# isl-org/Open3D-ML

Hardware: AMD Instinct MI355X
Metric: point-cloud frames/sec (RandLA-Net SemanticKITTI inference: H2D + kNN pyramid + forward) (higher is better)
Workload: dtype f32

## Files before the change

open3d-ml_amd/csrc/grid.h:

```cpp
#pragma once
#include <hip/hip_runtime.h>
#include <stdint.h>

namespace ml3d {

constexpr int GRID_CAP = 8;
constexpr int GRID_SLACK = 64;
constexpr int GRID_LEVELS = 5;

struct Segs {
    const int64_t* splits;
    int64_t stride;
    int64_t n_uniform;
    int batch;
};

struct GridSeg {
    float lo[3];
    float c, inv_c;
    float margin;
    int dims[3];
    int cell_base;
    int n;
    int sorted_base;
    float c0;
    int dims0[3];
    float ext[3];
    float dim_est;
    int probe_stride;
};

struct GridView {
    const GridSeg* segs;
    const int* cell_start;
    const float4* sorted;
    int batch;
};

struct GridWs {
    GridSeg* segs;
    unsigned* bbox;
    unsigned* occ;
    unsigned* bitmap;
    int* cells;
    int* block_sums;
    float4* sorted;
    int64_t total_cells;
    int64_t bitmap_words;
    int64_t n_total;
    int batch;
};

constexpr int GRID_SORTED_SLACK = 4;
size_t grid_ws_bytes(int64_t n_total, int64_t batch);
bool grid_ws_carve(void* ws, size_t bytes, int64_t n_total, int64_t batch, GridWs* out);
int grid_build(const float* points, Segs segs, const GridWs& ws, float target_occ, hipStream_t stream);
int grid_build_derived(const float* points, Segs segs, const GridWs& ws, const GridWs& parent, hipStream_t stream);
int grid_build_fixed(const float* points, Segs segs, const GridWs& ws, float cell, hipStream_t stream);
int bbox_compute(const float* points, Segs segs, int64_t n_total, unsigned* bbox, unsigned* occ_scratch,
                 hipStream_t stream);
int scan_inclusive_i32(int* a, int64_t n, int* block_sums, hipStream_t stream);

void zero_async(void* ptr, size_t bytes, hipStream_t stream);

__device__ __forceinline__ unsigned f2ord(float f) {
    unsigned u = __float_as_uint(f);
    return (u & 0x80000000u) ? ~u : (u | 0x80000000u);
}
__device__ __forceinline__ float ord2f(unsigned u) {
    return __uint_as_float((u & 0x80000000u) ? (u & 0x7fffffffu) : ~u);
}

__device__ __forceinline__ void wave_sync() {
    __threadfence_block();
    __builtin_amdgcn_wave_barrier();
}

__device__ __forceinline__ void wave_lds_sync() {
    __builtin_amdgcn_fence(__ATOMIC_RELEASE, "wavefront");
    __builtin_amdgcn_wave_barrier();
    __builtin_amdgcn_fence(__ATOMIC_ACQUIRE, "wavefront");
}


__device__ __forceinline__ float fmax_raw(float a, float b) { return __builtin_amdgcn_fmed3f(a, b, 3.0e38f); }

__device__ __forceinline__ int wave_inclusive_scan(int v) {
    const int lane = threadIdx.x & 63;
#pragma unroll
    for (int o = 1; o < 64; o <<= 1) {
        int u = __shfl_up(v, o);
        if (lane >= o) v += u;
    }
    return v;
}
__device__ __forceinline__ int wave_sum(int v) {
#pragma unroll
    for (int o = 32; o > 0; o >>= 1) v += __shfl_xor(v, o);
    return v;
}

__device__ __forceinline__ void block_sync_lds() {
    __builtin_amdgcn_fence(__ATOMIC_RELEASE, "workgroup", "local");
    __builtin_amdgcn_s_barrier();
    __builtin_amdgcn_fence(__ATOMIC_ACQUIRE, "workgroup", "local");
}

inline GridView grid_view(const GridWs& ws) {
    GridView v;
    v.segs = ws.segs;
    v.cell_start = ws.cells;
    v.sorted = ws.sorted;
    v.batch = ws.batch;
    return v;
}


__device__ __forceinline__ int64_t seg_begin_global(const Segs& S, int s) {
    return S.splits ? S.splits[s] : (int64_t)s * S.stride;
}
__device__ __forceinline__ int64_t seg_begin_packed(const Segs& S, int s) {
    return S.splits ? S.splits[s] : (int64_t)s * S.n_uniform;
}
__device__ __forceinline__ int64_t seg_len(const Segs& S, int s) {
    return S.splits ? (S.splits[s + 1] - S.splits[s]) : S.n_uniform;
}
__device__ __forceinline__ void seg_locate(const Segs& S, int64_t packed, int& s, int64_t& local) {
    if (!S.splits) {
        s = (int)(packed / S.n_uniform);
        local = packed - (int64_t)s * S.n_uniform;
        return;
    }
    int lo = 0, hi = S.batch;
    while (hi - lo > 1) {
        int mid = (lo + hi) >> 1;
        if (S.splits[mid] <= packed) lo = mid; else hi = mid;
    }
    s = lo;
    local = packed - S.splits[lo];
}
// ... 42 lines not shown
```

open3d-ml_amd/csrc/grid.hip:

```cpp
#include "grid.h"

#include <math.h>

namespace ml3d {

static inline size_t align_up(size_t x) { return (x + 255) & ~(size_t)255; }

static void grid_sizes(int64_t n_total, int64_t batch, int64_t* total_cells, int64_t* bitmap_words,
                       int64_t* n_blocks) {
    *total_cells = (int64_t)GRID_CAP * n_total + (int64_t)GRID_SLACK * batch;
    *bitmap_words = (*total_cells + 31) / 32 + batch;
    *n_blocks = (*total_cells + 2 + 1023) / 1024 + 1;
}

size_t grid_ws_bytes(int64_t n_total, int64_t batch) {
    int64_t tc, bw, nb;
    grid_sizes(n_total, batch, &tc, &bw, &nb);
    size_t b = 0;
    b += align_up(sizeof(GridSeg) * (size_t)batch);
    b += align_up(sizeof(unsigned) * 6 * (size_t)batch);
    b += align_up(sizeof(unsigned) * GRID_LEVELS * (size_t)batch);
    b += align_up(sizeof(unsigned) * GRID_LEVELS * (size_t)bw);
    b += align_up(sizeof(int) * (size_t)(tc + 2));
    b += align_up(sizeof(int) * (size_t)nb);
// ... 221 lines not shown
        const int64_t last = first + blockDim.x - 1 < total ? first + blockDim.x - 1 : total - 1;
        s0 = (int)(first / per); s1 = (int)(last / per);
    } else {
        const int64_t last = first + blockDim.x - 1 < n_total ? first + blockDim.x - 1 : n_total - 1;
        seg_locate_wave(S, first, s0, l0);
        seg_locate_wave(S, last, s1, l1);
    }
    const bool one_item = (s0 == s1);
    if (threadIdx.x < GRID_LEVELS) cnt[threadIdx.x] = 0u;
    __syncthreads();
    const int64_t i = first + threadIdx.x;
    bool valid;
    int s = s0; int64_t local = l0 + threadIdx.x;
    if (dense_stride > 0) {
        s = (int)(i / per);
        local = (i - (int64_t)s * per) * dense_stride;
        valid = s < S.batch && local < S.n_uniform;
        if (!valid) s = s0;
    } else {
        valid = i < n_total;
        if (valid && !one_item) seg_locate(S, i, s, local);
    }
    int cx = 0, cy = 0, cz = 0;
    const GridSeg* g = &segs[s];
    valid = valid && (local % g->probe_stride == 0);
    if (valid) {
        const float* p = pts + 3 * (seg_begin_global(S, s) + local);
        float inv = 1.0f / g->c0;
        cx = cell_coord(p[0], g->lo[0], inv, g->dims0[0]);
        cy = cell_coord(p[1], g->lo[1], inv, g->dims0[1]);
        cz = cell_coord(p[2], g->lo[2], inv, g->dims0[2]);
    }
    const int64_t bit_base = (int64_t)g->cell_base + 32 * (int64_t)s;
    for (int l = 0; l < GRID_LEVELS; ++l) {
        bool fresh = false;
        if (valid) {
            int dx = ((g->dims0[0] - 1) >> l) + 1, dy = ((g->dims0[1] - 1) >> l) + 1;
            int64_t id = (cx >> l) + (int64_t)dx * ((cy >> l) + (int64_t)dy * (cz >> l));
            int64_t bit = bit_base + id;
            unsigned m = 1u << (unsigned)(bit & 31);
            unsigned old = atomicOr(&bitmap[(int64_t)l * bitmap_words + (bit >> 5)], m);
            fresh = !(old & m);
        }
        if (one_item) {
            unsigned long long b = __ballot(fresh);
            if ((threadIdx.x & 63) == 0 && b) atomicAdd(&cnt[l], (unsigned)__popcll(b));
        } else if (fresh) {
            atomicAdd(&occ[GRID_LEVELS * s + l], 1u);
        }
    }
    __syncthreads();
    if (one_item && threadIdx.x < GRID_LEVELS && cnt[threadIdx.x])
        atomicAdd(&occ[GRID_LEVELS * s0 + threadIdx.x], cnt[threadIdx.x]);
}

__device__ __forceinline__ float occ_of_lam(float lam) { return lam / (1.0f - expf(-lam)); }
__device__ __forceinline__ float lam_of_occ(float m) {
    if (m <= 1.0005f) return 1.0e-3f;
    float lo = 1.0e-3f, hi = 64.0f;
    if (m >= hi) return m;
    for (int it = 0; it < 40; ++it) {
        float mid = 0.5f * (lo + hi);
        if (occ_of_lam(mid) < m) lo = mid; else hi = mid;
    }
    return 0.5f * (lo + hi);
}

__device__ __forceinline__ void finish_grid(GridSeg& g, float c, int64_t cap) {
    float emax = fmaxf(g.ext[0], fmaxf(g.ext[1], g.ext[2]));
    int d[3] = {1, 1, 1};
    if (emax > 0.f) {
        for (int it = 0; it < 200; ++it) {
            if (dims_fit(g.ext, c, cap, d)) break;
            c *= 1.1f;
        }
    } else {
        c = 1.0f;
    }
    g.c = c;
    g.inv_c = 1.0f / c;
    for (int a = 0; a < 3; ++a) g.dims[a] = d[a];
}

__global__ void grid_setup1(const unsigned* occ, GridSeg* segs, int batch, float target) {
    int s = blockIdx.x * blockDim.x + threadIdx.x;
    if (s >= batch) return;
    GridSeg g = segs[s];
    int64_t n = g.n;
    float emax = fmaxf(g.ext[0], fmaxf(g.ext[1], g.ext[2]));
    int64_t cap = (int64_t)GRID_CAP * n + GRID_SLACK;
    float c = g.c0;
    if (n > 0 && emax > 0.f) {
        const float n_probe = (float)((n + g.probe_stride - 1) / g.probe_stride);
        const float lam_goal = lam_of_occ(target) / (float)g.probe_stride;
        float lam_prev = 0.f, lam_cur = 0.f;
        int lsel = -1;
        for (int l = 0; l < GRID_LEVELS; ++l) {
            unsigned cnt = occ[GRID_LEVELS * s + l];
            lam_cur = lam_of_occ(n_probe / (float)(cnt > 0u ? cnt : 1u));
            if (lam_cur >= lam_goal) { lsel = l; break; }
            lam_prev = lam_cur;
        }
        if (lsel == 0) {
            c = g.c0;
        } else if (lsel > 0) {
            float D = fminf(fmaxf(log2f(lam_cur / lam_prev), 1.0f), 3.0f);
            g.dim_est = D;
            c = g.c0 * (float)(1 << (lsel - 1)) * powf(lam_goal / lam_prev, 1.0f / D);
        } else {
            c = g.c0 * (float)(1 << (GRID_LEVELS - 1));
            if (n <= 64) c = emax * 2.0f;
        }
    }
    finish_grid(g, c, cap);
    segs[s] = g;
}

__global__ void grid_setup_derived(Segs S, const GridSeg* parent, GridSeg* segs, int batch) {
    int s = blockIdx.x * blockDim.x + threadIdx.x;
    if (s >= batch) return;
    GridSeg g = parent[s];
    int64_t n = seg_len(S, s);
    int64_t pb = seg_begin_packed(S, s);
    float ratio = n > 0 ? (float)g.n / (float)n : 1.0f;
    float c = g.c * powf(fmaxf(ratio, 1.0f), 1.0f / g.dim_est);
    g.n = (int)n;
    g.sorted_base = (int)pb;
    g.cell_base = (int)(GRID_CAP * pb + (int64_t)GRID_SLACK * s);
    if (n <= 64) c = fmaxf(g.ext[0], fmaxf(g.ext[1], g.ext[2])) * 2.0f;
    finish_grid(g, c, (int64_t)GRID_CAP * n + GRID_SLACK);
    segs[s] = g;
}

__device__ __forceinline__ int point_cell(const GridSeg* g, float x, float y, float z) {
    int cx = cell_coord(x, g->lo[0], g->inv_c, g->dims[0]);
    int cy = cell_coord(y, g->lo[1], g->inv_c, g->dims[1]);
    int cz = cell_coord(z, g->lo[2], g->inv_c, g->dims[2]);
    return g->cell_base + cx + g->dims[0] * (cy + g->dims[1] * cz);
}

__global__ void grid_hist(const float* __restrict__ pts, Segs S, int64_t n_total,
                          const GridSeg* __restrict__ segs, int* cells) {
    int64_t i = (int64_t)blockIdx.x * blockDim.x + threadIdx.x;
    if (i >= n_total) return;
    int s; int64_t local;
    seg_locate(S, i, s, local);
    const float* p = pts + 3 * (seg_begin_global(S, s) + local);
    int cid = point_cell(&segs[s], p[0], p[1], p[2]);
    atomicAdd(&cells[cid + 2], 1);
}

constexpr int SCAN_TILE = 4096;


__global__ void __launch_bounds__(256) scan_block_sums(const int* __restrict__ a, int64_t n, int* block_sums) {
    __shared__ int ws[4];
    const int64_t base = (int64_t)blockIdx.x * SCAN_TILE;
    int v = 0;
#pragma unroll
    for (int j = 0; j < SCAN_TILE / 256; ++j) {
        int64_t i = base + j * 256 + threadIdx.x;
        if (i < n) v += a[i];
    }
    v = wave_sum(v);
    if ((threadIdx.x & 63) == 0) ws[threadIdx.x >> 6] = v;
    __syncthreads();
    if (threadIdx.x == 0) block_sums[blockIdx.x] = ws[0] + ws[1] + ws[2] + ws[3];
}

__global__ void __launch_bounds__(1024) scan_sums(int* block_sums, int64_t nb) {
    __shared__ int wsum[16];
    const int t = threadIdx.x;
    const int64_t per = (nb + 1023) / 1024;
    const int64_t lo = (int64_t)t * per, hi = lo + per < nb ? lo + per : nb;
    int s = 0;
    for (int64_t i = lo; i < hi; ++i) s += block_sums[i];
    int incl = wave_inclusive_scan(s);
    if ((t & 63) == 63) wsum[t >> 6] = incl;
    __syncthreads();
    int carry = 0;
    for (int w = 0; w < (t >> 6); ++w) carry += wsum[w];
    int run = carry + incl - s;
    for (int64_t i = lo; i < hi; ++i) {
        int v = block_sums[i];
        block_sums[i] = run;
        run += v;
    }
}

__global__ void __launch_bounds__(256) scan_final(int* a, int64_t n, const int* __restrict__ block_sums) {
    __shared__ int ws[4];
    const int lane = threadIdx.x & 63, wv = threadIdx.x >> 6;
    const int64_t base = (int64_t)blockIdx.x * SCAN_TILE + (int64_t)wv * 1024;
    int v[16], tot = 0;
#pragma unroll
    for (int r = 0; r < 16; ++r) {
        int64_t i = base + r * 64 + lane;
        v[r] = i < n ? a[i] : 0;
        tot += v[r];
    }
    tot = wave_sum(tot);
    if (lane == 0) ws[wv] = tot;
    __syncthreads();
    int carry = block_sums[blockIdx.x];
    for (int w = 0; w < wv; ++w) carry += ws[w];
#pragma unroll
    for (int r = 0; r < 16; ++r) {
        int incl = wave_inclusive_scan(v[r]) + carry;
        int64_t i = base + r * 64 + lane;
        if (i < n) a[i] = incl;
        carry = __shfl(incl, 63);
    }
}

// ... 74 lines not shown
    return 0;
}

static int grid_sort(const float* points, Segs S, const GridWs& ws, hipStream_t stream) {
    int64_t n = ws.n_total;
    int nb = (int)((n + 255) / 256);
    if (n > 0) {
        hipLaunchKernelGGL(grid_hist, dim3(nb), dim3(256), 0, stream, points, S, n, ws.segs, ws.cells);
        ML3D_LAUNCH_CHECK();
        if (scan_inclusive_i32(ws.cells + 2, ws.total_cells, ws.block_sums, stream)) return -3;
        hipLaunchKernelGGL(grid_scatter, dim3(nb), dim3(256), 0, stream, points, S, n, ws.segs, ws.cells,
                           ws.sorted);
        ML3D_LAUNCH_CHECK();
    }
    return 0;
}


int grid_build(const float* points, Segs S, const GridWs& ws, float target_occ, hipStream_t stream) {
    int64_t n = ws.n_total;
    int B = ws.batch;
    if (B <= 0) return 0;
    if (target_occ <= 0.f) target_occ = 4.0f;
    int sb = (B + 63) / 64;
    zero_async(ws.bitmap, (size_t)((char*)(ws.cells + ws.total_cells + 2) - (char*)ws.bitmap), stream);
    hipLaunchKernelGGL(grid_bbox_init, dim3(sb), dim3(64), 0, stream, ws.bbox, ws.occ, B);
    ML3D_LAUNCH_CHECK();
    if (n > 0) {
        int nb4 = (int)((n + 1023) / 1024);
        hipLaunchKernelGGL(grid_bbox, dim3(nb4), dim3(256), 0, stream, points, S, n, ws.bbox);
        ML3D_LAUNCH_CHECK();
    }
    hipLaunchKernelGGL(grid_setup0, dim3(sb), dim3(64), 0, stream, S, ws.bbox, ws.segs, B);
    ML3D_LAUNCH_CHECK();
    int nb = (int)((n + 255) / 256);
    if (n > 0) {
        const int dense = (!S.splits && S.n_uniform >= 32768) ? 16 : 0;
        const int nbo = dense ? (int)((((S.n_uniform + dense - 1) / dense) * (int64_t)S.batch + 255) / 256) : nb;
        hipLaunchKernelGGL(grid_occupancy, dim3(nbo), dim3(256), 0, stream, points, S, n, ws.segs, ws.bitmap,
                           ws.bitmap_words, ws.occ, dense);
        ML3D_LAUNCH_CHECK();
    }
    hipLaunchKernelGGL(grid_setup1, dim3(sb), dim3(64), 0, stream, ws.occ, ws.segs, B, target_occ);
    ML3D_LAUNCH_CHECK();
    return grid_sort(points, S, ws, stream);
}

__global__ void grid_setup_fixed(GridSeg* segs, int batch, float cell) {
    int s = blockIdx.x * blockDim.x + threadIdx.x;
    if (s >= batch) return;
    GridSeg g = segs[s];
    float c = cell;
    if (!(c > 0.f)) c = g.c0;
    if (c < g.c0 * 0.5f) c = g.c0 * 0.5f;
    finish_grid(g, c, (int64_t)GRID_CAP * g.n + GRID_SLACK);
    segs[s] = g;
}

int bbox_compute(const float* points, Segs S, int64_t n, unsigned* bbox, unsigned* occ_scratch, hipStream_t stream) {
    int B = S.batch;
    if (B <= 0) return 0;
    hipLaunchKernelGGL(grid_bbox_init, dim3((B + 63) / 64), dim3(64), 0, stream, bbox, occ_scratch, B);
    ML3D_LAUNCH_CHECK();
    if (n > 0) {
        hipLaunchKernelGGL(grid_bbox, dim3((unsigned)((n + 1023) / 1024)), dim3(256), 0, stream, points, S, n, bbox);
        ML3D_LAUNCH_CHECK();
    }
    return 0;
}

int grid_build_fixed(const float* points, Segs S, const GridWs& ws, float cell, hipStream_t stream) {
    int B = ws.batch;
    if (B <= 0) return 0;
    int sb = (B + 63) / 64;
    zero_async(ws.cells, sizeof(int) * (size_t)(ws.total_cells + 2), stream);
    if (bbox_compute(points, S, ws.n_total, ws.bbox, ws.occ, stream)) return -3;
    hipLaunchKernelGGL(grid_setup0, dim3(sb), dim3(64), 0, stream, S, ws.bbox, ws.segs, B);
    ML3D_LAUNCH_CHECK();
    hipLaunchKernelGGL(grid_setup_fixed, dim3(sb), dim3(64), 0, stream, ws.segs, B, cell);
    ML3D_LAUNCH_CHECK();
    return grid_sort(points, S, ws, stream);
}

int grid_build_derived(const float* points, Segs S, const GridWs& ws, const GridWs& parent, hipStream_t stream) {
    int B = ws.batch;
    if (B <= 0) return 0;
    zero_async(ws.cells, sizeof(int) * (size_t)(ws.total_cells + 2), stream);
    hipLaunchKernelGGL(grid_setup_derived, dim3((B + 63) / 64), dim3(64), 0, stream, S, parent.segs, ws.segs, B);
    ML3D_LAUNCH_CHECK();
    return grid_sort(points, S, ws, stream);
}

}
```

open3d-ml_amd/csrc/knn.hip:

```cpp
#include <hip/hip_runtime.h>
#include <stdint.h>
#include <stdlib.h>

#include <gfx950_ops.h>

#include "grid.h"
#include "ml3d_hip.h"

namespace ml3d {

typedef unsigned long long u64;
constexpr u64 KEY_EMPTY = 0x7ff0000000000000ull;

struct QuerySrc {
    const float4* sorted_q;
    const GridSeg* qsegs;
    const float* raw;
    Segs segs;
    int64_t n_total;
};

template <int K>
__device__ __forceinline__ void topk_insert(double (&best)[K], double key) {
    if (key < best[K - 1]) {
// ... 142 lines not shown
        };
        float dk = 3.0e38f;
        int r_in = 0, r = 1;
        if constexpr (MODE == 2) {
#pragma unroll
            for (int j = 0; j < K; ++j) best[j] = H->keys[(size_t)j * H->cap + hslot];
            best1 = H->keys[(size_t)K * H->cap + hslot];
            u64 kth0;
            dk = known_within(kth0);
            r_in = 1; r = 2;
        }
        for (;;) {
            scan_shell<K, SUB>(G, g, qx, qy, qz, cx, cy, cz, r_in, r, dk, best, n_sub, best1);
            bool all;
            const float gd = shell_guard(g, qx, qy, qz, cx, cy, cz, r, all);
            if (all) break;
            u64 kth;
            dk = known_within(kth);
            if (kth != KEY_EMPTY && gd > 0.f && dk < gd * gd * 0.999999f) break;
            if constexpr (MODE == 1) {
                if (r == 1) {
                    const unsigned slot = wave_append(H->count);
                    if (slot < H->cap) {
#pragma unroll
                        for (int j = 0; j < K; ++j) H->keys[(size_t)j * H->cap + slot] = best[j];
                        H->keys[(size_t)K * H->cap + slot] = best1;
                        H->who[slot] = (job << 28) | (uint32_t)t;
                        return;
                    }
                }
            }
            r_in = r;
            if (r < UNIT_SHELLS) { ++r; continue; }
            int rn = r + max(1, r >> 1);
            if (dk < 3.0e38f) {
                const float rad = sqrtf(dk) * 1.00001f + g.margin;
                const int need = max(max(cx - cell_coord(qx - rad, g.lo[0], g.inv_c, g.dims[0]), cell_coord(qx + rad, g.lo[0], g.inv_c, g.dims[0]) - cx),
                                     max(max(cy - cell_coord(qy - rad, g.lo[1], g.inv_c, g.dims[1]), cell_coord(qy + rad, g.lo[1], g.inv_c, g.dims[1]) - cy),
                                         max(cz - cell_coord(qz - rad, g.lo[2], g.inv_c, g.dims[2]), cell_coord(qz + rad, g.lo[2], g.inv_c, g.dims[2]) - cz)));
                rn = max(r + 1, need);
            }
            r = rn;
        }
    }
    int64_t base = index_local ? 0 : seg_begin_global(support_segs, s);
    if (SUB) {
        const u64 k1 = (u64)__double_as_longlong(best1);
        out_sub[out_row] = k1 != KEY_EMPTY ? (int32_t)(unsigned)(k1 & 0xffffffffull) : -1;
    }
    if (K == 16 && k == 16 && !out_d2 && vec_store) {
        struct alignas(16) I4 { int32_t v[4]; };
        I4* dst = reinterpret_cast<I4*>(out_idx + out_row * 16);
#pragma unroll
        for (int qd = 0; qd < 4; ++qd) {
            I4 o;
#pragma unroll
            for (int e = 0; e < 4; ++e) {
                const u64 key = (u64)__double_as_longlong(best[4 * qd + e]);
                o.v[e] = key != KEY_EMPTY ? (int32_t)((int64_t)(unsigned)(key & 0xffffffffull) + base) : -1;
            }
            dst[qd] = o;
        }
        return;
    }
#pragma unroll
    for (int j = 0; j < K; ++j) {
        if (j < k) {
            u64 key = (u64)__double_as_longlong(best[j]);
            bool ok = key != KEY_EMPTY;
            out_idx[out_row * k + j] = ok ? (int32_t)((int64_t)(unsigned)(key & 0xffffffffull) + base) : -1;
            if (out_d2) out_d2[out_row * k + j] = ok ? __uint_as_float((unsigned)(key >> 32)) : __uint_as_float(0x7f800000u);
        }
    }
}

template <int K>
__global__ void __launch_bounds__(256)
knn_query(GridView G, QuerySrc Q, int k, int index_local, Segs support_segs, int32_t* __restrict__ out_idx,
          float* __restrict__ out_d2) {
    knn_one<K, false>(G, Q, k, index_local, support_segs, out_idx, out_d2, (int64_t)blockIdx.x * blockDim.x + threadIdx.x);
}

constexpr int KNN_MAX_JOBS = 8;
struct KnnJob {
    GridView G;
    QuerySrc Q;
    Segs support;
    int32_t* out_idx;
    int32_t* out_sub;
    int n_sub;
    unsigned block_begin;
};
struct KnnJobs {
    KnnJob j[KNN_MAX_JOBS];
    int n;
};

#ifndef KNN_WAVES
#define KNN_WAVES 5
#endif
template <int K, bool SUB, bool HAND>
__global__ void __launch_bounds__(256)
#if KNN_WAVES > 0
ML3D_WAVES_PER_SIMD(KNN_WAVES)
#endif
knn_query_multi(KnnJobs J, int k, int index_local, int vec_store, Handoff H) {
    int ji = 0;
#pragma unroll
    for (int i = 1; i < KNN_MAX_JOBS; ++i)
        if (i < J.n && blockIdx.x >= J.j[i].block_begin) ji = i;
    const KnnJob& jb = J.j[ji];
    knn_one<K, SUB, HAND ? 1 : 0>(jb.G, jb.Q, k, index_local, jb.support, jb.out_idx, nullptr,
                                  (int64_t)(blockIdx.x - jb.block_begin) * blockDim.x + threadIdx.x, jb.n_sub, jb.out_sub, vec_store != 0,
                                  &H, (unsigned)ji);
}

#ifndef KNN_WAVES_HAND
#define KNN_WAVES_HAND 4
#endif
template <int K, bool SUB>
__global__ void __launch_bounds__(256)
ML3D_WAVES_PER_SIMD(KNN_WAVES_HAND)
knn_first(KnnJobs J, int k, int index_local, int vec_store, Handoff H) {
    int ji = 0;
#pragma unroll
    for (int i = 1; i < KNN_MAX_JOBS; ++i)
        if (i < J.n && blockIdx.x >= J.j[i].block_begin) ji = i;
    const KnnJob& jb = J.j[ji];
    knn_one<K, SUB, 1>(jb.G, jb.Q, k, index_local, jb.support, jb.out_idx, nullptr,
                       (int64_t)(blockIdx.x - jb.block_begin) * blockDim.x + threadIdx.x, jb.n_sub, jb.out_sub, vec_store != 0, &H, (unsigned)ji);
}

template <int K, bool SUB>
__global__ void __launch_bounds__(256)
ML3D_WAVES_PER_SIMD(KNN_WAVES_HAND)
knn_continue(KnnJobs J, int k, int index_local, int vec_store, Handoff H) {
    const unsigned have = *H.count;
    const unsigned n = have < H.cap ? have : H.cap;
    const unsigned i = blockIdx.x * blockDim.x + threadIdx.x;
    if (i >= n) return;
    const uint32_t who = H.who[i];
    const KnnJob& jb = J.j[who >> 28];
    knn_one<K, SUB, 2>(jb.G, jb.Q, k, index_local, jb.support, jb.out_idx, nullptr, (int64_t)(who & 0x0fffffffu), jb.n_sub, jb.out_sub,
                       vec_store != 0, &H, who >> 28, i);
}

static int knn_block() { return 64; }

static size_t handoff_bytes(int64_t total_queries) {
    const size_t cap = (size_t)(total_queries * 5 / 8 + 64);
    return 256 + ((cap * 4 + 255) & ~(size_t)255) + 17 * cap * 8 + 256;
}
static Handoff handoff_carve(char* p, int64_t total_queries) {
    Handoff H;
    const size_t cap = (size_t)(total_queries * 5 / 8 + 64);
    p = (char*)(((uintptr_t)p + 255) & ~(uintptr_t)255);
    H.count = (unsigned*)p;  p += 256;
    H.who = (uint32_t*)p;    p += (cap * 4 + 255) & ~(size_t)255;
    H.keys = (double*)p;
    H.cap = (unsigned)cap;
    return H;
}

#ifndef ML3D_KNN_HANDOFF
#define ML3D_KNN_HANDOFF 0
#endif

template <bool SUB>
static int launch_query_multi(KnnJobs& J, int k, int index_local, hipStream_t stream, const Handoff* hand = nullptr) {
    const int T = knn_block();
    unsigned blocks = 0;
    int vec = 1;
    for (int i = 0; i < J.n; ++i) {
        J.j[i].block_begin = blocks;
        blocks += (unsigned)((J.j[i].Q.n_total + T - 1) / T);
        if ((uintptr_t)J.j[i].out_idx & 15) vec = 0;
    }
    if (blocks == 0) return 0;
    Handoff H = {};
    if ((ML3D_KNN_HANDOFF) && hand && k > 8 && k <= 16) {
        H = *hand;
        zero_async(H.count, 16, stream);
        hipLaunchKernelGGL((knn_first<16, SUB>), dim3(blocks), dim3(T), 0, stream, J, k, index_local, vec, H);
        if (hipGetLastError() != hipSuccess) return ML3D_E_LAUNCH;
        hipLaunchKernelGGL((knn_continue<16, SUB>), dim3((H.cap + T - 1) / T), dim3(T), 0, stream, J, k, index_local, vec, H);
        return hipGetLastError() == hipSuccess ? 0 : ML3D_E_LAUNCH;
    }
    if (k == 1) hipLaunchKernelGGL((knn_query_multi<1, SUB, false>), dim3(blocks), dim3(T), 0, stream, J, k, index_local, vec, H);
    else if (k <= 8) hipLaunchKernelGGL((knn_query_multi<8, SUB, false>), dim3(blocks), dim3(T), 0, stream, J, k, index_local, vec, H);
    else if (k <= 16) hipLaunchKernelGGL((knn_query_multi<16, SUB, false>), dim3(blocks), dim3(T), 0, stream, J, k, index_local, vec, H);
    else if (k <= 32) hipLaunchKernelGGL((knn_query_multi<32, SUB, false>), dim3(blocks), dim3(T), 0, stream, J, k, index_local, vec, H);
    else if (k <= 64) hipLaunchKernelGGL((knn_query_multi<64, SUB, false>), dim3(blocks), dim3(T), 0, stream, J, k, index_local, vec, H);
    else return ML3D_E_UNSUPPORTED;
    return hipGetLastError() == hipSuccess ? 0 : ML3D_E_LAUNCH;
}

static int launch_query(const GridView& G, const QuerySrc& Q, int k, int index_local, Segs support_segs,
                        int32_t* out_idx, float* out_d2, hipStream_t stream) {
    if (Q.n_total <= 0) return 0;
    dim3 grid((unsigned)((Q.n_total + 255) / 256)), block(256);
    if (k == 1)
        hipLaunchKernelGGL(knn_query<1>, grid, block, 0, stream, G, Q, k, index_local, support_segs, out_idx, out_d2);
    else if (k <= 8)
        hipLaunchKernelGGL(knn_query<8>, grid, block, 0, stream, G, Q, k, index_local, support_segs, out_idx, out_d2);
    else if (k <= 16)
        hipLaunchKernelGGL(knn_query<16>, grid, block, 0, stream, G, Q, k, index_local, support_segs, out_idx, out_d2);
    else if (k <= 32)
        hipLaunchKernelGGL(knn_query<32>, grid, block, 0, stream, G, Q, k, index_local, support_segs, out_idx, out_d2);
    else if (k <= 64)
        hipLaunchKernelGGL(knn_query<64>, grid, block, 0, stream, G, Q, k, index_local, support_segs, out_idx, out_d2);
    else
        return ML3D_E_UNSUPPORTED;
    return hipGetLastError() == hipSuccess ? 0 : ML3D_E_LAUNCH;
}

__global__ void order_from_grid(const float4* __restrict__ sorted, int64_t n_total, int64_t n_per_item,
                                int32_t* __restrict__ out) {
    const int64_t i = (int64_t)blockIdx.x * blockDim.x + threadIdx.x;
    if (i >= n_total) return;
    out[i] = (int32_t)((i / n_per_item) * n_per_item + (int64_t)__float_as_int(sorted[i].w));
}

static constexpr float tuning_occ() { return 0.f; }

}

using namespace ml3d;

extern "C" int ml3d_abi_version(void) { return ML3D_ABI_VERSION; }

extern "C" size_t ml3d_knn_workspace_bytes(int64_t n_points, int64_t n_queries, int64_t batch) {
    (void)n_queries;
    return grid_ws_bytes(n_points, batch);
}

extern "C" int ml3d_knn_search(const float* points, const int64_t* points_row_splits, const float* queries,
                               const int64_t* queries_row_splits, int64_t batch, int64_t n_points,
                               int64_t n_queries, int k, int index_local, int32_t* out_index,
                               float* out_dist2, void* workspace, size_t workspace_bytes, void* stream) {
    if (!points_row_splits || !queries_row_splits || batch <= 0 || k <= 0 || n_points < 0 || n_queries < 0 ||
        n_points > 0x7fffffffll / GRID_CAP - 4096 || n_queries > 0x7fffffffll)
        return ML3D_E_INVALID;
    if (k > 64) return ML3D_E_UNSUPPORTED;
    if (n_queries == 0) return 0;
    if (!out_index || (n_points > 0 && !points) || !queries) return ML3D_E_INVALID;
    GridWs ws;
    if (!grid_ws_carve(workspace, workspace_bytes, n_points, batch, &ws)) return ML3D_E_WORKSPACE;
    hipStream_t st = (hipStream_t)stream;
    Segs ps = {points_row_splits, 0, 0, (int)batch};
    Segs qs = {queries_row_splits, 0, 0, (int)batch};
    int rc = grid_build(points, ps, ws, tuning_occ(), st);
    if (rc) return ML3D_E_LAUNCH;
    GridView G = grid_view(ws);
    QuerySrc Q;
    bool self = (queries == points) && (queries_row_splits == points_row_splits) && (n_queries == n_points);
    Q.sorted_q = self ? ws.sorted : nullptr;
    Q.qsegs = ws.segs;
    Q.raw = queries;
    Q.segs = qs;
    Q.n_total = n_queries;
    return launch_query(G, Q, k, index_local, ps, out_index, out_dist2, st);
}

static int pyramid_sizes(int64_t n0, int num_layers, const int32_t* ratios, int64_t* n ) {
    n[0] = n0;
    for (int l = 0; l < num_layers; ++l) {
        if (ratios[l] <= 0) return -1;
        n[l + 1] = n[l] / ratios[l];
    }
    return 0;
}

extern "C" size_t ml3d_randla_pyramid_workspace_bytes(int64_t batch, int64_t n0, int num_layers,
                                                      const int32_t* ratios_host) {
    if (num_layers <= 0 || num_layers > KNN_MAX_JOBS || !ratios_host) return 0;
    int64_t n[17];
    if (pyramid_sizes(n0, num_layers, ratios_host, n)) return 0;
    size_t b = 0;
    int64_t total = 0;
    for (int l = 0; l < num_layers; ++l) { b += grid_ws_bytes(n[l] * batch, batch) + 256; total += n[l] * batch; }
    return b + handoff_bytes(total);
}

extern "C" int ml3d_randla_knn_pyramid(const float* points, int64_t batch, int64_t n0, int num_layers,
                                       const int32_t* ratios_host, int k, int32_t* const* neighbor_idx_host,
                                       int32_t* const* interp_idx_host, void* workspace, size_t workspace_bytes,
                                       void* stream) {
    return ml3d_randla_knn_pyramid_traced(points, batch, n0, num_layers, ratios_host, k, neighbor_idx_host,
                                          interp_idx_host, workspace, workspace_bytes, stream, nullptr);
}

extern "C" int ml3d_randla_knn_pyramid_traced(const float* points, int64_t batch, int64_t n0, int num_layers,
                                              const int32_t* ratios_host, int k,
                                              int32_t* const* neighbor_idx_host, int32_t* const* interp_idx_host,
                                              void* workspace, size_t workspace_bytes, void* stream,
                                              const ml3d_trace* tr) {
    return ml3d_randla_knn_pyramid_ordered(points, batch, n0, num_layers, ratios_host, k, neighbor_idx_host,
                                           interp_idx_host, nullptr, workspace, workspace_bytes, stream, tr);
}

extern "C" int ml3d_randla_knn_pyramid_ordered(const float* points, int64_t batch, int64_t n0, int num_layers,
                                               const int32_t* ratios_host, int k,
                                               int32_t* const* neighbor_idx_host, int32_t* const* interp_idx_host,
                                               int32_t* const* tile_order_host, void* workspace,
                                               size_t workspace_bytes, void* stream, const ml3d_trace* tr) {
    auto tb = [&](int tag) { for (const ml3d_trace* r = tr; r; r = r->next) if (r->tag == tag && r->ev_start) (void)hipEventRecord((hipEvent_t)r->ev_start, (hipStream_t)stream); };
    auto te = [&](int tag) { for (const ml3d_trace* r = tr; r; r = r->next) if (r->tag == tag && r->ev_stop) (void)hipEventRecord((hipEvent_t)r->ev_stop, (hipStream_t)stream); };
    if (!points || batch <= 0 || n0 <= 0 || num_layers <= 0 || num_layers > KNN_MAX_JOBS || !ratios_host || k <= 0 ||
        !neighbor_idx_host || !interp_idx_host)
        return ML3D_E_INVALID;
    if (k > 64) return ML3D_E_UNSUPPORTED;
    int64_t n[17];
    if (pyramid_sizes(n0, num_layers, ratios_host, n)) return ML3D_E_INVALID;
    if (n0 * batch > 0x7fffffffll / GRID_CAP - 4096) return ML3D_E_INVALID;
    if (workspace_bytes < ml3d_randla_pyramid_workspace_bytes(batch, n0, num_layers, ratios_host))
        return ML3D_E_WORKSPACE;
    hipStream_t st = (hipStream_t)stream;
    GridWs ws[17];
    char* p = (char*)workspace;
    for (int l = 0; l < num_layers; ++l) {
        size_t bytes = grid_ws_bytes(n[l] * batch, batch) + 256;
        if (!grid_ws_carve(p, bytes, n[l] * batch, batch, &ws[l])) return ML3D_E_WORKSPACE;
        p += bytes;
    }
    float occ = tuning_occ();
    for (int l = 0; l < num_layers; ++l) {
        if (n[l] == 0) continue;
        Segs S = {nullptr, n0, n[l], (int)batch};
        tb(100 + l);
        if (l == 0 ? grid_build(points, S, ws[l], occ, st) : grid_build_derived(points, S, ws[l], ws[0], st))
            return ML3D_E_LAUNCH;
        if (tile_order_host && tile_order_host[l]) {
            const int64_t nt = n[l] * batch;
            hipLaunchKernelGGL(order_from_grid, dim3((unsigned)((nt + 255) / 256)), dim3(256), 0, st, ws[l].sorted, nt, n[l],
                               tile_order_host[l]);
            if (hipGetLastError() != hipSuccess) return ML3D_E_LAUNCH;
        }
        te(100 + l);
    }
    KnnJobs Jk;
    Jk.n = 0;
    for (int l = 0; l < num_layers; ++l) {
        if (n[l] == 0) continue;
        Segs S = {nullptr, n0, n[l], (int)batch};
        QuerySrc Q;
        Q.sorted_q = ws[l].sorted;
        Q.qsegs = ws[l].segs;
        Q.raw = points;
        Q.segs = S;
        Q.n_total = n[l] * batch;
        KnnJob& a = Jk.j[Jk.n++];
        a.G = grid_view(ws[l]); a.Q = Q; a.support = S; a.out_idx = neighbor_idx_host[l]; a.block_begin = 0;
        a.out_sub = interp_idx_host[l];
        a.n_sub = (int)n[l + 1];
    }
    int64_t total_q = 0;
    for (int l = 0; l < num_layers; ++l) total_q += n[l] * batch;
    const Handoff hand = handoff_carve(p, total_q);
    tb(0);
    int rc = launch_query_multi<true>(Jk, k, 1, st, &hand);
    te(0);
    return rc;
}

#include <hip/hip_fp16.h>

#include "sort.h"

namespace ml3d {

__global__ void center_keys(const float* __restrict__ pts, int64_t n, double cx, double cy, double cz,
                            const float* __restrict__ cdev, u64* __restrict__ keys, uint32_t* __restrict__ vals) {
    const int64_t i = (int64_t)blockIdx.x * blockDim.x + threadIdx.x;
    if (i >= n) return;
    if (cdev) { cx = (double)cdev[0]; cy = (double)cdev[1]; cz = (double)cdev[2]; }
    const double dx = (double)pts[3 * i] - cx, dy = (double)pts[3 * i + 1] - cy, dz = (double)pts[3 * i + 2] - cz;
    const double d2 = (dx * dx + dy * dy) + dz * dz;
    keys[i] = (u64)__double_as_longlong(d2);
    vals[i] = (uint32_t)i;
}

__global__ void center_take(const u64* __restrict__ keys, const uint32_t* __restrict__ vals, int64_t k,
                            int32_t* __restrict__ out_idx, double* __restrict__ out_d2) {
    const int64_t i = (int64_t)blockIdx.x * blockDim.x + threadIdx.x;
    if (i >= k) return;
    out_idx[i] = (int32_t)vals[i];
    if (out_d2) out_d2[i] = __longlong_as_double((long long)keys[i]);
}

__global__ void __launch_bounds__(256)
vote_update(const float* __restrict__ logits, const int32_t* __restrict__ inds, int64_t n, int C, float smooth,
            __half* __restrict__ probs, int64_t n_cloud) {
    const int lane = threadIdx.x & 63;
    const int64_t i = (int64_t)blockIdx.x * 4 + (threadIdx.x >> 6);
    if (i >= n) return;
    const float* row = logits + i * C;
    float mx = -3.0e38f;
    for (int c = lane; c < C; c += 64) mx = fmaxf(mx, row[c]);
#pragma unroll
    for (int o = 32; o > 0; o >>= 1) mx = fmaxf(mx, __shfl_xor(mx, o));
    float sum = 0.f;
    for (int c = lane; c < C; c += 64) sum += expf(row[c] - mx);
#pragma unroll
    for (int o = 32; o > 0; o >>= 1) sum += __shfl_xor(sum, o);
    const int64_t dst = inds[i];
    if (dst < 0 || dst >= n_cloud) return;
    const __half hs = __float2half(smooth);
    const float w_new = 1.0f - smooth;
    for (int c = lane; c < C; c += 64) {
        const float p = expf(row[c] - mx) / sum;
        const __half old = probs[dst * C + c];
        const __half keep = __float2half(__half2float(hs) * __half2float(old));
        probs[dst * C + c] = __float2half(__half2float(keep) + w_new * p);
    }
}

__global__ void __launch_bounds__(256)
argmax_rows(const float* __restrict__ scores, int64_t n, int C, uint8_t* __restrict__ out) {
    const int64_t i = (int64_t)blockIdx.x * blockDim.x + threadIdx.x;
    if (i >= n) return;
    const float* row = scores + i * C;
    float best = row[0];
    int arg = 0;
    for (int c = 1; c < C; ++c) {
        const float v = row[c];
        if ((v > best || v != v) && !(best != best)) { best = v; arg = c; }
    }
    out[i] = (uint8_t)arg;
}

__global__ void __launch_bounds__(64)
argmax_rows_lds(const float* __restrict__ scores, int64_t n, int C, uint8_t* __restrict__ out) {
    __shared__ __attribute__((aligned(16))) float tile[64 * 32];
    const int64_t r0 = (int64_t)blockIdx.x * 64;
    const int rows = (int)((n - r0) < 64 ? (n - r0) : 64);
    const int64_t f0 = r0 * C;
    const int total = rows * C;
    const float* src = scores + f0;
    const int mis = (int)(f0 & 3);
    const int head = mis ? 4 - mis : 0;
    for (int e = threadIdx.x; e < head && e < total; e += 64) tile[e] = src[e];
    const int n4 = total > head ? (total - head) / 4 : 0;
    const float4* s4 = reinterpret_cast<const float4*>(src + head);
// ... 226 lines not shown
```

Measured before the change: 7558.

## Build all kNN pyramid grids in one fused multi-level pass

Measured after the change: 7562 (median of 2 runs). Within noise of the previous version (+0.0%).

```diff
diff --git a/open3d-ml_amd/csrc/grid.h b/open3d-ml_amd/csrc/grid.h
--- a/open3d-ml_amd/csrc/grid.h
+++ b/open3d-ml_amd/csrc/grid.h
@@ -55,7 +55,9 @@
 size_t grid_ws_bytes(int64_t n_total, int64_t batch);
 bool grid_ws_carve(void* ws, size_t bytes, int64_t n_total, int64_t batch, GridWs* out);
 int grid_build(const float* points, Segs segs, const GridWs& ws, float target_occ, hipStream_t stream);
-int grid_build_derived(const float* points, Segs segs, const GridWs& ws, const GridWs& parent, hipStream_t stream);
+constexpr int GRID_MAX_LEVELS = 8;
+int grid_build_pyramid(const float* points, const int64_t* n, int num_levels, int batch, const GridWs* ws,
+                       int32_t* const* tile_order, float target_occ, hipStream_t stream);
 int grid_build_fixed(const float* points, Segs segs, const GridWs& ws, float cell, hipStream_t stream);
 int bbox_compute(const float* points, Segs segs, int64_t n_total, unsigned* bbox, unsigned* occ_scratch,
                  hipStream_t stream);
diff --git a/open3d-ml_amd/csrc/grid.hip b/open3d-ml_amd/csrc/grid.hip
--- a/open3d-ml_amd/csrc/grid.hip
+++ b/open3d-ml_amd/csrc/grid.hip
@@ -327,10 +327,7 @@
     for (int a = 0; a < 3; ++a) g.dims[a] = d[a];
 }
 
-__global__ void grid_setup1(const unsigned* occ, GridSeg* segs, int batch, float target) {
-    int s = blockIdx.x * blockDim.x + threadIdx.x;
-    if (s >= batch) return;
-    GridSeg g = segs[s];
+__device__ __forceinline__ void setup1_item(const unsigned* occ, GridSeg& g, int s, float target) {
     int64_t n = g.n;
     float emax = fmaxf(g.ext[0], fmaxf(g.ext[1], g.ext[2]));
     int64_t cap = (int64_t)GRID_CAP * n + GRID_SLACK;
@@ -358,15 +355,17 @@
         }
     }
     finish_grid(g, c, cap);
-    segs[s] = g;
-}
-
-__global__ void grid_setup_derived(Segs S, const GridSeg* parent, GridSeg* segs, int batch) {
+}
+
+__global__ void grid_setup1(const unsigned* occ, GridSeg* segs, int batch, float target) {
     int s = blockIdx.x * blockDim.x + threadIdx.x;
     if (s >= batch) return;
-    GridSeg g = parent[s];
-    int64_t n = seg_len(S, s);
-    int64_t pb = seg_begin_packed(S, s);
+    GridSeg g = segs[s];
+    setup1_item(occ, g, s, target);
+    segs[s] = g;
+}
+
+__device__ __forceinline__ void derived_item(GridSeg& g, int64_t n, int64_t pb, int s) {
     float ratio = n > 0 ? (float)g.n / (float)n : 1.0f;
     float c = g.c * powf(fmaxf(ratio, 1.0f), 1.0f / g.dim_est);
     g.n = (int)n;
@@ -374,7 +373,6 @@
     g.cell_base = (int)(GRID_CAP * pb + (int64_t)GRID_SLACK * s);
     if (n <= 64) c = fmaxf(g.ext[0], fmaxf(g.ext[1], g.ext[2])) * 2.0f;
     finish_grid(g, c, (int64_t)GRID_CAP * n + GRID_SLACK);
-    segs[s] = g;
 }
 
 __device__ __forceinline__ int point_cell(const GridSeg* g, float x, float y, float z) {
@@ -615,13 +613,214 @@
     return grid_sort(points, S, ws, stream);
 }
 
-int grid_build_derived(const float* points, Segs S, const GridWs& ws, const GridWs& parent, hipStream_t stream) {
-    int B = ws.batch;
-    if (B <= 0) return 0;
-    zero_async(ws.cells, sizeof(int) * (size_t)(ws.total_cells + 2), stream);
-    hipLaunchKernelGGL(grid_setup_derived, dim3((B + 63) / 64), dim3(64), 0, stream, S, parent.segs, ws.segs, B);
-    ML3D_LAUNCH_CHECK();
-    return grid_sort(points, S, ws, stream);
-}
-
-}
+struct GridLevels {
+    GridSeg* segs[GRID_MAX_LEVELS];
+    int* cells[GRID_MAX_LEVELS];
+    float4* sorted[GRID_MAX_LEVELS];
+    int32_t* order[GRID_MAX_LEVELS];
+    int n[GRID_MAX_LEVELS];
+    unsigned zero_begin[GRID_MAX_LEVELS];
+    unsigned zero_per[GRID_MAX_LEVELS];
+    int nl, batch;
+};
+
+__device__ __forceinline__ int seg_used_cells(const GridSeg& g) { return g.dims[0] * g.dims[1] * g.dims[2]; }
+
+__global__ void grid_setup_levels(GridLevels L, const unsigned* occ, float target) {
+    int s = blockIdx.x * blockDim.x + threadIdx.x;
+    if (s >= L.batch) return;
+    GridSeg g0 = L.segs[0][s];
+    setup1_item(occ, g0, s, target);
+    L.segs[0][s] = g0;
+    for (int l = 1; l < L.nl; ++l) {
+        GridSeg g = g0;
+        derived_item(g, L.n[l], (int64_t)s * L.n[l], s);
+        L.segs[l][s] = g;
+    }
+}
+
+constexpr int ZERO_WORDS = 4096;
+__global__ void __launch_bounds__(256)
+grid_zero_bitmap(const GridSeg* __restrict__ segs, unsigned* __restrict__ bitmap, int64_t bitmap_words, unsigned chunks) {
+    const unsigned sl = blockIdx.x / chunks, chunk = blockIdx.x % chunks;
+    const int s = (int)(sl / GRID_LEVELS), l = (int)(sl % GRID_LEVELS);
+    const GridSeg* g = &segs[s];
+    const int64_t bits = (int64_t)(((g->dims0[0] - 1) >> l) + 1) * (((g->dims0[1] - 1) >> l) + 1) * (((g->dims0[2] - 1) >> l) + 1);
+    const int64_t bit_base = (int64_t)g->cell_base + 32 * (int64_t)s;
+    const int64_t w0 = bit_base >> 5, w1 = (bit_base + bits - 1) >> 5;
+    const int64_t first = w0 + (int64_t)chunk * ZERO_WORDS;
+    if (first > w1) return;
+    unsigned* p = bitmap + (int64_t)l * bitmap_words;
+#pragma unroll
+    for (int j = 0; j < ZERO_WORDS / 256; ++j) {
+        const int64_t w = first + j * 256 + threadIdx.x;
+        if (w <= w1) p[w] = 0u;
+    }
+}
+
+__global__ void __launch_bounds__(256) grid_zero_cells(GridLevels L) {
+    int l = 0;
+#pragma unroll
+    for (int i = 1; i < GRID_MAX_LEVELS; ++i)
+        if (i < L.nl && blockIdx.x >= L.zero_begin[i]) l = i;
+    const unsigned rel = blockIdx.x - L.zero_begin[l];
+    const int s = (int)(rel / L.zero_per[l]);
+    const int chunk = (int)(rel % L.zero_per[l]);
+    const GridSeg* g = &L.segs[l][s];
+    const int len = seg_used_cells(*g) + 2;
+    if (chunk * ZERO_WORDS >= len) return;
+    int* a = L.cells[l] + g->cell_base;
+#pragma unroll
+    for (int j = 0; j < ZERO_WORDS / 1024; ++j) {
+        const int w = chunk * ZERO_WORDS + 4 * (j * 256 + (int)threadIdx.x);
+        if (w + 4 <= len) {
+            *(uint4*)(a + w) = make_uint4(0u, 0u, 0u, 0u);
+        } else {
+            for (int q = w; q < len; ++q) a[q] = 0;
+        }
+    }
+}
+
+__global__ void __launch_bounds__(256) grid_hist_levels(const float* __restrict__ pts, GridLevels L) {
+    const int64_t i = (int64_t)blockIdx.x * blockDim.x + threadIdx.x;
+    const int n0 = L.n[0];
+    if (i >= (int64_t)n0 * L.batch) return;
+    const int s = (int)(i / n0), local = (int)(i - (int64_t)s * n0);
+    const float* p = pts + 3 * i;
+    const float x = p[0], y = p[1], z = p[2];
+#pragma unroll
+    for (int l = 0; l < GRID_MAX_LEVELS; ++l)
+        if (l < L.nl && local < L.n[l]) atomicAdd(&L.cells[l][point_cell(&L.segs[l][s], x, y, z) + 2], 1);
+}
+
+__global__ void __launch_bounds__(1024) grid_scan_items(GridLevels L) {
+    __shared__ int ws[16];
+    const int l = blockIdx.x / L.batch, s = blockIdx.x % L.batch;
+    const int lane = threadIdx.x & 63, wv = threadIdx.x >> 6;
+    const GridSeg* g = &L.segs[l][s];
+    const int used = seg_used_cells(*g);
+    const int first_slot = g->sorted_base;
+    int* a = L.cells[l] + g->cell_base + 2;
+    if (threadIdx.x == 0) {
+        int reach = 0;
+        if (s > 0) {
+            const GridSeg* gp = &L.segs[l][s - 1];
+            reach = seg_used_cells(*gp) + 2 - (g->cell_base - gp->cell_base);
+        }
+        if (reach < 1) a[-2] = first_slot;
+        if (reach < 2) a[-1] = first_slot;
+    }
+    const int rows = (used + 1023) / 1024;
+    const int base = wv * rows * 64;
+    int tot = 0;
+    for (int r = 0; r < rows; r += 4) {
+        int v[4];
+#pragma unroll
+        for (int q = 0; q < 4; ++q) {
+            const int i = base + (r + q) * 64 + lane;
+            v[q] = (r + q < rows && i < used) ? a[i] : 0;
+        }
+        tot += (v[0] + v[1]) + (v[2] + v[3]);
+    }
+    tot = wave_sum(tot);
+    if (lane == 0) ws[wv] = tot;
+    __syncthreads();
+    int carry = first_slot;
+    for (int w = 0; w < wv; ++w) carry += ws[w];
+    for (int r = 0; r < rows; r += 4) {
+        int v[4];
+#pragma unroll
+        for (int q = 0; q < 4; ++q) {
+            const int i = base + (r + q) * 64 + lane;
+            v[q] = (r + q < rows && i < used) ? a[i] : 0;
+        }
+#pragma unroll
+        for (int q = 0; q < 4; ++q) {
+            const int i = base + (r + q) * 64 + lane;
+            const int incl = wave_inclusive_scan(v[q]) + carry;
+            if (r + q < rows && i < used) a[i] = incl;
+            carry = __shfl(incl, 63);
+        }
+    }
+}
+
+__global__ void __launch_bounds__(256) grid_scatter_levels(const float* __restrict__ pts, GridLevels L) {
+    const int64_t i = (int64_t)blockIdx.x * blockDim.x + threadIdx.x;
+    const int n0 = L.n[0];
+    if (i >= (int64_t)n0 * L.batch) return;
+    const int s = (int)(i / n0), local = (int)(i - (int64_t)s * n0);
+    const float* p = pts + 3 * i;
+    const float x = p[0], y = p[1], z = p[2];
+    const float4 e = make_float4(x, y, z, __int_as_float(local));
+    int pos[GRID_MAX_LEVELS];
+#pragma unroll
+    for (int l = 0; l < GRID_MAX_LEVELS; ++l)
+        if (l < L.nl && local < L.n[l]) pos[l] = atomicAdd(&L.cells[l][point_cell(&L.segs[l][s], x, y, z) + 1], 1);
+#pragma unroll
+    for (int l = 0; l < GRID_MAX_LEVELS; ++l) {
+        if (l < L.nl && local < L.n[l]) {
+            L.sorted[l][pos[l]] = e;
+            if (L.order[l]) L.order[l][pos[l]] = s * L.n[l] + local;
+        }
+    }
+}
+
+int grid_build_pyramid(const float* points, const int64_t* n, int num_levels, int batch, const GridWs* ws,
+                       int32_t* const* tile_order, float target_occ, hipStream_t stream) {
+    if (batch <= 0 || num_levels <= 0) return 0;
+    if (num_levels > GRID_MAX_LEVELS || n[0] <= 0) return -3;
+    if (target_occ <= 0.f) target_occ = 4.0f;
+    const int B = batch, sb = (B + 63) / 64;
+    const int64_t nt = n[0] * B;
+    GridLevels L;
+    L.nl = num_levels;
+    L.batch = B;
+    unsigned zero_blocks = 0;
+    for (int l = 0; l < GRID_MAX_LEVELS; ++l) {
+        const bool on = l < num_levels;
+        if (on && (n[l] <= 0 || (l > 0 && n[l] > n[l - 1]) || ws[l].batch != B || ws[l].n_total != n[l] * B)) return -3;
+        L.segs[l] = on ? ws[l].segs : nullptr;
+        L.cells[l] = on ? ws[l].cells : nullptr;
+        L.sorted[l] = on ? ws[l].sorted : nullptr;
+        L.order[l] = on && tile_order ? tile_order[l] : nullptr;
+        L.n[l] = on ? (int)n[l] : 0;
+        L.zero_begin[l] = zero_blocks;
+        L.zero_per[l] = on ? (unsigned)(((int64_t)GRID_CAP * n[l] + GRID_SLACK + 2 + ZERO_WORDS - 1) / ZERO_WORDS) : 1u;
+        if (on) zero_blocks += L.zero_per[l] * (unsigned)B;
+    }
+    const GridWs& w0 = ws[0];
+    const Segs S = {nullptr, n[0], n[0], B};
+    hipLaunchKernelGGL(grid_bbox_init, dim3(sb), dim3(64), 0, stream, w0.bbox, w0.occ, B);
+    ML3D_LAUNCH_CHECK();
+    hipLaunchKernelGGL(grid_bbox, dim3((unsigned)((nt + 1023) / 1024)), dim3(256), 0, stream, points, S, nt, w0.bbox);
+    ML3D_LAUNCH_CHECK();
+    hipLaunchKernelGGL(grid_setup0, dim3(sb), dim3(64), 0, stream, S, w0.bbox, w0.segs, B);
+    ML3D_LAUNCH_CHECK();
+    {
+        const int64_t words = ((int64_t)GRID_CAP * n[0] + GRID_SLACK + 31) / 32 + 1;
+        const unsigned chunks = (unsigned)((words + ZERO_WORDS - 1) / ZERO_WORDS);
+        hipLaunchKernelGGL(grid_zero_bitmap, dim3(chunks * (unsigned)(B * GRID_LEVELS)), dim3(256), 0, stream, w0.segs, w0.bitmap,
+                           w0.bitmap_words, chunks);
+        ML3D_LAUNCH_CHECK();
+    }
+    {
+        const int dense = n[0] >= 32768 ? 16 : 0;
+        const int64_t threads = dense ? ((n[0] + dense - 1) / dense) * (int64_t)B : nt;
+        hipLaunchKernelGGL(grid_occupancy, dim3((unsigned)((threads + 255) / 256)), dim3(256), 0, stream, points, S, nt, w0.segs,
+                           w0.bitmap, w0.bitmap_words, w0.occ, dense);
+        ML3D_LAUNCH_CHECK();
+    }
+    hipLaunchKernelGGL(grid_setup_levels, dim3(sb), dim3(64), 0, stream, L, w0.occ, target_occ);
+    ML3D_LAUNCH_CHECK();
+    hipLaunchKernelGGL(grid_zero_cells, dim3(zero_blocks), dim3(256), 0, stream, L);
+    ML3D_LAUNCH_CHECK();
+    hipLaunchKernelGGL(grid_hist_levels, dim3((unsigned)((nt + 255) / 256)), dim3(256), 0, stream, points, L);
+    ML3D_LAUNCH_CHECK();
+    hipLaunchKernelGGL(grid_scan_items, dim3((unsigned)(num_levels * B)), dim3(1024), 0, stream, L);
+    ML3D_LAUNCH_CHECK();
+    hipLaunchKernelGGL(grid_scatter_levels, dim3((unsigned)((nt + 255) / 256)), dim3(256), 0, stream, points, L);
+    ML3D_LAUNCH_CHECK();
+    return 0;
+}
+
+}
diff --git a/open3d-ml_amd/csrc/knn.hip b/open3d-ml_amd/csrc/knn.hip
--- a/open3d-ml_amd/csrc/knn.hip
+++ b/open3d-ml_amd/csrc/knn.hip
@@ -248,6 +248,7 @@
 }
 
 constexpr int KNN_MAX_JOBS = 8;
+static_assert(KNN_MAX_JOBS == GRID_MAX_LEVELS, "the pyramid builds one grid per search job (grid_build_pyramid)");
 struct KnnJob {
     GridView G;
     QuerySrc Q;
@@ -378,13 +379,6 @@
     else
         return ML3D_E_UNSUPPORTED;
     return hipGetLastError() == hipSuccess ? 0 : ML3D_E_LAUNCH;
-}
-
-__global__ void order_from_grid(const float4* __restrict__ sorted, int64_t n_total, int64_t n_per_item,
-                                int32_t* __restrict__ out) {
-    const int64_t i = (int64_t)blockIdx.x * blockDim.x + threadIdx.x;
-    if (i >= n_total) return;
-    out[i] = (int32_t)((i / n_per_item) * n_per_item + (int64_t)__float_as_int(sorted[i].w));
 }
 
 static constexpr float tuning_occ() { return 0.f; }
@@ -445,7 +439,11 @@
     size_t b = 0;
     int64_t total = 0;
     for (int l = 0; l < num_layers; ++l) { b += grid_ws_bytes(n[l] * batch, batch) + 256; total += n[l] * batch; }
-    return b + handoff_bytes(total);
+#if ML3D_KNN_HANDOFF
+    b += handoff_bytes(total);
+#endif
+    (void)total;
+    return b;
 }
 
 extern "C" int ml3d_randla_knn_pyramid(const float* points, int64_t batch, int64_t n0, int num_layers,
@@ -489,21 +487,12 @@
         if (!grid_ws_carve(p, bytes, n[l] * batch, batch, &ws[l])) return ML3D_E_WORKSPACE;
         p += bytes;
     }
-    float occ = tuning_occ();
-    for (int l = 0; l < num_layers; ++l) {
-        if (n[l] == 0) continue;
-        Segs S = {nullptr, n0, n[l], (int)batch};
-        tb(100 + l);
-        if (l == 0 ? grid_build(points, S, ws[l], occ, st) : grid_build_derived(points, S, ws[l], ws[0], st))
-            return ML3D_E_LAUNCH;
-        if (tile_order_host && tile_order_host[l]) {
-            const int64_t nt = n[l] * batch;
-            hipLaunchKernelGGL(order_from_grid, dim3((unsigned)((nt + 255) / 256)), dim3(256), 0, st, ws[l].sorted, nt, n[l],
-                               tile_order_host[l]);
-            if (hipGetLastError() != hipSuccess) return ML3D_E_LAUNCH;
-        }
-        te(100 + l);
-    }
+    int nla = 0;
+    while (nla < num_layers && n[nla] > 0) ++nla;
+    tb(100);
+    if (grid_build_pyramid(points, n, nla, (int)batch, ws, tile_order_host, tuning_occ(), st)) return ML3D_E_LAUNCH;
+    te(100);
+    for (int l = 1; l < nla; ++l) { tb(100 + l); te(100 + l); }
     KnnJobs Jk;
     Jk.n = 0;
     for (int l = 0; l < num_layers; ++l) {
@@ -522,9 +511,15 @@
     }
     int64_t total_q = 0;
     for (int l = 0; l < num_layers; ++l) total_q += n[l] * batch;
+#if ML3D_KNN_HANDOFF
     const Handoff hand = handoff_carve(p, total_q);
+    const Handoff* hp = &hand;
+#else
+    const Handoff* hp = nullptr;
+    (void)total_q;
+#endif
     tb(0);
-    int rc = launch_query_multi<true>(Jk, k, 1, st, &hand);
+    int rc = launch_query_multi<true>(Jk, k, 1, st, hp);
     te(0);
     return rc;
 }
```
